# finalfusion/reductive

Hardware: AMD Instinct MI355X
Metric: vectors/sec PQ encode (d=300, M=15, K=256) (higher is better)
Workload: dtype f32

## Files before the change

reductive_amd/csrc/kernels_mfma16_screen.hip.h:

```cpp
#pragma once
#include "kernels_mfma.hip.h"

namespace pqhip {

constexpr float kScreenRel = 0x1.2p-9f;
constexpr float kScreenAbs = 0x1p-100f;
constexpr float kScreenTiny = 0x1p-100f;
constexpr int kScreenScaleLo = 12;
constexpr float kScreenMaxXX = 0x1p30f;
constexpr float kScreenMinCC = 0x1p-100f;

template <int T, int DP> constexpr bool mfma16_screens() { return mfma16_screen_shape(T, DP); }

constexpr int kScreenImageBytes = 256 * 32 * 2;
constexpr int kScreenHeaderBytes = 16;
constexpr size_t screen_image_bytes(int64_t M) { return (size_t)M * (kScreenImageBytes + kScreenHeaderBytes); }

struct ScreenScale {
    bool cc_range;
    float sc, sc2;
};
__device__ __forceinline__ ScreenScale screen_scale(float maxcc)
{
    ScreenScale r;
    r.cc_range = maxcc >= kScreenMinCC && maxcc < kBigNorm;
    const int escale = r.cc_range ? (kScreenScaleLo + 1 - ((int)(__float_as_uint(maxcc) >> 23) - 127)) >> 1 : 0;
    r.sc = __uint_as_float((unsigned)(127 + escale) << 23);
    r.sc2 = __uint_as_float((unsigned)(127 + 2 * escale) << 23);
    return r;
}

typedef _Float16 f16x8_t __attribute__((ext_vector_type(8)));
typedef _Float16 f16x2_t __attribute__((ext_vector_type(2)));
typedef unsigned u32x4_t __attribute__((ext_vector_type(4)));

__device__ __forceinline__ unsigned pk_f16(float a, float b)
{
    return __builtin_bit_cast(unsigned, __builtin_convertvector((f32x2){a, b}, f16x2_t));
}
__device__ __forceinline__ float f16_lo(unsigned p) { return (float)__builtin_bit_cast(f16x2_t, p)[0]; }
__device__ __forceinline__ float vmin(float a, float b) { float r; asm("v_min_f32 %0, %1, %2" : "=v"(r) : "v"(a), "v"(b)); return r; }
__device__ __forceinline__ float vmax(float a, float b) { float r; asm("v_max_f32 %0, %1, %2" : "=v"(r) : "v"(a), "v"(b)); return r; }
__device__ __forceinline__ void keep2(float& m, float& s, float k1, float k2)
{
    float t;
    asm("v_med3_f32 %0, %1, %2, %3" : "=v"(t) : "v"(m), "v"(k1), "v"(k2));
    asm("v_min_f32 %0, %0, %1" : "+v"(s) : "v"(t));
    asm("v_min3_f32 %0, %0, %1, %2" : "+v"(m) : "v"(k1), "v"(k2));
}
__device__ __forceinline__ float vmin3(float a, float b, float c) { float r; asm("v_min3_f32 %0, %1, %2, %3" : "=v"(r) : "v"(a), "v"(b), "v"(c)); return r; }
__device__ __forceinline__ void fold2(float& m, float a, float b) { asm("v_min3_f32 %0, %0, %1, %2" : "+v"(m) : "v"(a), "v"(b)); }

#define PQHIP_GLOBAL_AS __attribute__((address_space(1)))
#define PQHIP_LDS_AS __attribute__((address_space(3)))
typedef unsigned u32x2_t __attribute__((ext_vector_type(2)));
typedef f32x4_u PQHIP_GLOBAL_AS const* gf32x4_p;
__device__ __forceinline__ void load20_global(const PQHIP_GLOBAL_AS float* p, float (&v)[20])
{
#pragma unroll
    for (int e = 0; e < 20; e += 4) {
        const f32x4 t = *reinterpret_cast<gf32x4_p>(p + e);
        v[e] = t[0]; v[e + 1] = t[1]; v[e + 2] = t[2]; v[e + 3] = t[3];
    }
}
__device__ __forceinline__ float chain_dot20(const float (&a)[20], const float (&b)[20])
{
    float ab = 0.f;
#pragma unroll
    for (int k = 0; k < 20; ++k) ab = ffma(a[k], b[k], ab);
    return ab;
}

template <typename IdxT>
__device__ __forceinline__ void encode_rows_cand_f16(const float* x, int64_t x_rs, void* out, int64_t o_rs, const float* cbk,
                                                  const float* ccn, int K, int k_pad, int dsub, int64_t n, int m,
                                                  int64_t row_begin, const unsigned short* img, const unsigned* tiles,
                                                  unsigned long long flagged_c, float sc, float maxcct)
{
    constexpr int DP = 20, kRow = 32;
    const int lane = threadIdx.x & 63;
    const int i16 = lane & 15;
    const int q = lane >> 4;
    const int c0 = (8 * q) % 20, c1 = (8 * q + 4) % 20;
    const PQHIP_GLOBAL_AS float* const xsub = (const PQHIP_GLOBAL_AS float*)x + (int64_t)m * dsub;
    const PQHIP_GLOBAL_AS float* const plast = xsub + (n - 1) * x_rs;
    const PQHIP_GLOBAL_AS float* const cbm = (const PQHIP_GLOBAL_AS float*)cbk + (int64_t)m * K * DP;
    const PQHIP_GLOBAL_AS float* const ccm = (const PQHIP_GLOBAL_AS float*)ccn + (int64_t)m * k_pad;
    const PQHIP_LDS_AS unsigned* const tiles_l = (const PQHIP_LDS_AS unsigned*)tiles;
    const float sl = q < 3 ? sc : 0.f;
    const float sc2 = sc * sc;
    const PQHIP_LDS_AS unsigned short* const arow = (const PQHIP_LDS_AS unsigned short*)img + (i16 * kRow + 8 * (q ^ ((i16 >> 2) & 3)));
    unsigned cur = 0;
    int cur_ti = 0;
    while (cur || flagged_c) {
        int rel = -1;
        for (int t = 0; t < 16; ++t) {
            while (!cur && flagged_c) {
                cur_ti = __builtin_ctzll(flagged_c);
                flagged_c &= flagged_c - 1;
                cur = __builtin_amdgcn_readfirstlane(tiles_l[cur_ti]);
            }
            if (!cur) break;
            const int r = 32 * cur_ti + __builtin_ctz(cur);
            cur &= cur - 1;
            if (i16 == t) rel = r;
        }
        const bool rv = rel >= 0;
        const int64_t row = row_begin + rel;
        const PQHIP_GLOBAL_AS float* p = rv ? xsub + row * x_rs : plast;
        const f32x4 v0 = *reinterpret_cast<gf32x4_p>(p + c0), v1 = *reinterpret_cast<gf32x4_p>(p + c1);
        unsigned w[4] = {pk_f16(sl * v0[0], sl * v0[1]), pk_f16(sl * v0[2], sl * v0[3]), pk_f16(sl * v1[0], sl * v1[1]),
                         pk_f16(sl * v1[2], sl * v1[3])};
        if (q == 2) { w[2] = 0x3c003c00u; w[3] = 0x7bffu; }
        const u32x4_t bo = (u32x4_t){w[0], w[1], w[2], w[3]};
        float s0 = 0.f, s1 = 0.f;
#pragma unroll
        for (int j = 0; j < 4; ++j) { s0 = fmaf(v0[j], v0[j], s0); s1 = fmaf(v1[j], v1[j], s1); }
        float u[4];
        gather_groups((q < 3 ? s0 : 0.f) + (q < 2 ? s1 : 0.f), u);
        const float xxs = sc2 * ((u[0] + u[1]) + (u[2] + u[3]));
        auto block = [&](const PQHIP_LDS_AS unsigned short* ar, int cb) {
            const u32x4_t af = *reinterpret_cast<const PQHIP_LDS_AS u32x4_t*>(ar + cb * 16 * kRow);
            return __builtin_amdgcn_mfma_f32_16x16x32_f16(__builtin_bit_cast(f16x8_t, af), __builtin_bit_cast(f16x8_t, bo),
                                                          (f32x4){0.f, 0.f, 0.f, 0.f}, 0, 0, 0);
        };
        float mn = __builtin_inff();
#pragma unroll
        for (int cb = 0; cb < 16; ++cb) {
            if (cb % 4 == 0) __builtin_amdgcn_sched_barrier(0);
            const f32x4 d = block(arow, cb);
            mn = __builtin_elementwise_minimum(mn, __builtin_elementwise_minimum(__builtin_elementwise_minimum(d[0], d[1]),
                                                                                 __builtin_elementwise_minimum(d[2], d[3])));
        }
        float mq[4];
        gather_groups(mn, mq);
        const float tau = rv ? fminf(fminf(mq[0], mq[1]), fminf(mq[2], mq[3])) + (kScreenRel * (xxs + maxcct) + kScreenAbs)
                             : __builtin_nanf("");
        const PQHIP_LDS_AS unsigned short* arow2 = arow;
        asm volatile("" : "+v"(arow2) : "v"(tau));
        unsigned cw[2] = {0u, 0u};
#pragma unroll
        for (int cb = 0; cb < 16; ++cb) {
            if (cb % 4 == 0) __builtin_amdgcn_sched_barrier(0);
            const f32x4 d = block(arow2, cb);
#pragma unroll
            for (int v = 0; v < 4; ++v) cw[cb >> 3] |= (d[v] <= tau ? 1u : 0u) << (4 * (cb & 7) + v);
            if (cb % 4 == 3) asm volatile("" : "+v"(cw[cb >> 3]));
        }
        unsigned long long cm = ((unsigned long long)cw[1] << 32) | cw[0];
        float xr[DP];
        load20_global(xsub + (rv ? row : 0) * x_rs, xr);
        const float xxe = rv ? norm_unrolled_static<DP>(xr) : 0.f;
        unsigned bh = 0xffffffffu, bl = 0xffffffffu;
        while (__builtin_amdgcn_ballot_w64(cm != 0)) {
            int j[2];
            bool cv[2];
            float ce[2][DP], ccj[2];
#pragma unroll
            for (int s = 0; s < 2; ++s) {
                const int bit = cm ? __builtin_ctzll(cm) : 0;
                j[s] = 16 * (bit >> 2) + 4 * q + (bit & 3);
                cv[s] = cm != 0 && j[s] < K;
                cm &= cm - 1;
                const int jj = cv[s] ? j[s] : 0;
                load20_global(cbm + (int64_t)jj * DP, ce[s]);
                ccj[s] = ccm[jj];
            }
#pragma unroll
            for (int s = 0; s < 2; ++s) {
                const float dp = chain_dot20(xr, ce[s]);
                const unsigned kh = ord_key(fsub(fadd(xxe, ccj[s]), fadd(dp, dp)));
                if (cv[s] && (kh < bh || (kh == bh && (unsigned)j[s] < bl))) { bh = kh; bl = (unsigned)j[s]; }
            }
        }
        float hq[4], lq[4];
        gather_groups(__uint_as_float(bh), hq);
        gather_groups(__uint_as_float(bl), lq);
        bh = __float_as_uint(hq[0]);
        bl = __float_as_uint(lq[0]);
#pragma unroll
        for (int g = 1; g < 4; ++g) {
            const unsigned h = __float_as_uint(hq[g]), l = __float_as_uint(lq[g]);
            if (h < bh || (h == bh && l < bl)) { bh = h; bl = l; }
        }
        if (rv && q == 0) ((PQHIP_GLOBAL_AS IdxT*)out)[row * o_rs + m] = (IdxT)bl;
    }
}

constexpr int kScreenFewCap = 96;
constexpr int kScreenFewWords = 3;

template <typename IdxT>
__device__ __noinline__ void encode_rows_few(const float* x, int64_t x_rs, void* out, int64_t o_rs, const float* cbk,
                                             const float* ccn, int K, int k_pad, int dsub, int m, int64_t row_begin,
                                             const uint2* list, int count)
{
    constexpr int DP = 20;
    const int lane = threadIdx.x & 63;
    const PQHIP_GLOBAL_AS float* const xsub = (const PQHIP_GLOBAL_AS float*)x + (int64_t)m * dsub;
    const PQHIP_GLOBAL_AS float* const cbm = (const PQHIP_GLOBAL_AS float*)cbk + (int64_t)m * K * DP;
    const PQHIP_GLOBAL_AS float* const ccm = (const PQHIP_GLOBAL_AS float*)ccn + (int64_t)m * k_pad;
    const PQHIP_LDS_AS u32x2_t* const list_l = (const PQHIP_LDS_AS u32x2_t*)list;
    for (int e0 = 0; e0 < count; e0 += 64) {
        const bool rv = e0 + lane < count;
        const PQHIP_LDS_AS u32x2_t* const en = list_l + kScreenFewWords * (rv ? e0 + lane : 0);
        const u32x2_t w0 = en[0], w1 = en[1], w2 = en[2];
        const unsigned key[4] = {w0[0], w0[1], w1[0], w1[1]};
        const float tau = __uint_as_float(w2[0]);
        const int64_t row = row_begin + w2[1];
        float xr[DP];
        load20_global(xsub + row * x_rs, xr);
        const float xxe = norm_unrolled_static<DP>(xr);
        unsigned bh = 0xffffffffu, bl = 0xffffffffu;
#pragma unroll
        for (int g = 0; g < 4; ++g) {
            const unsigned kb = key[g] & 63u;
            const int j = (int)(16u * (kb >> 2) + 4u * g + (kb & 3u));
            const bool cg = __uint_as_float(key[g]) <= tau && j < K;
            const int jj = cg ? j : 0;
            float ce[DP];
            load20_global(cbm + (int64_t)jj * DP, ce);
            const float dp = chain_dot20(xr, ce);
            const unsigned kh = ord_key(fsub(fadd(xxe, ccm[jj]), fadd(dp, dp)));
            if (cg && (kh < bh || (kh == bh && (unsigned)j < bl))) { bh = kh; bl = (unsigned)j; }
        }
        if (rv) ((PQHIP_GLOBAL_AS IdxT*)out)[row * o_rs + m] = (IdxT)bl;
    }
}

template <typename IdxT>
__device__ __forceinline__ void encode_mfma16_screen(const EncodeArgs& a)
{
    constexpr int DP = 20;
    constexpr int kRow = 32;
    __shared__ __attribute__((aligned(16))) unsigned short img_s[256 * kRow];
    __shared__ unsigned need_s[4][kMfma16MaxTiles];
    __shared__ unsigned cand_s[4][kMfma16MaxTiles];
    __shared__ uint2 few_s[4][kScreenFewCap * kScreenFewWords];

    const int lane = threadIdx.x & 63;
    const int wave = __builtin_amdgcn_readfirstlane(threadIdx.x >> 6);
    const int i16 = lane & 15;
    const int q = lane >> 4;

    const int64_t b = blockIdx.x;
    const int xcd = (int)(b & 7);
    const int64_t qq = b >> 3;
    const int64_t g_local = qq / a.M;
    const int m = (int)(qq - g_local * a.M);
    const int64_t group = g_local * 8 + xcd;
    const bool wg_active = (g_local < a.chunks_per_xcd) && (group < a.n_chunks);

    const unsigned long long st_s0 = a.stamps ? __builtin_amdgcn_s_memtime() : 0;
    unsigned maxcc_bits = 0u;
    if (wg_active) {
        const u32x4_t* src = reinterpret_cast<const u32x4_t*>(a.screen_img) + (int64_t)m * (kScreenImageBytes / 16) + threadIdx.x;
        u32x4_t* dst = reinterpret_cast<u32x4_t*>(img_s) + threadIdx.x;
        u32x4_t ch[4];
#pragma unroll
        for (int j = 0; j < 4; ++j) ch[j] = src[256 * j];
        maxcc_bits = a.screen_img[(int64_t)a.M * (kScreenImageBytes / 4) + m * (kScreenHeaderBytes / 4)];
#pragma unroll
        for (int j = 0; j < 4; ++j) dst[256 * j] = ch[j];
    }
    const float maxcc = __uint_as_float(maxcc_bits);
    const ScreenScale scale = screen_scale(maxcc);
    const bool cc_range = scale.cc_range;
    const float sc = scale.sc, sc2 = scale.sc2;
    __syncthreads();
    const unsigned long long st_stage = a.stamps ? __builtin_amdgcn_s_memtime() - st_s0 : 0;
    const int64_t row_begin = (group * 4 + wave) * a.rows_per_item;
    if (!wg_active || row_begin >= a.n) return;
    int64_t row_end = row_begin + a.rows_per_item;
    if (row_end > a.n) row_end = a.n;
    const bool bad_codebook = a.bad_flag != nullptr && *a.bad_flag != 0;
    const bool near_rows = (uint64_t)a.x_rs < (1ull << 24) && (uint64_t)a.o_rs < (1ull << 24);
    const bool cb_ok = !bad_codebook && cc_range && near_rows;
    const float maxcct = sc2 * maxcc;

    const int c0 = (8 * q) % 20, c1 = (8 * q + 4) % 20;
    const float* const xsub = a.x + (int64_t)m * a.dsub;
    const unsigned xrs4 = near_rows ? (unsigned)a.x_rs * 4u : 0u;
    const unsigned xoff0 = (unsigned)i16 * xrs4 + 4u * c0, xoff1 = (unsigned)i16 * xrs4 + 4u * c1;
    const unsigned ooff = near_rows ? (unsigned)lane * (unsigned)a.o_rs * (unsigned)sizeof(IdxT) : 0u;
    auto load_rows = [&](float (&v)[8], const char* base, unsigned o0, unsigned o1) {
        asm volatile("" : "+v"(o0), "+v"(o1));
        const f32x4 v0 = *reinterpret_cast<const f32x4_u*>(base + o0), v1 = *reinterpret_cast<const f32x4_u*>(base + o1);
#pragma unroll
        for (int j = 0; j < 4; ++j) { v[j] = v0[j]; v[4 + j] = v1[j]; }
    };
    auto load_tile = [&](float (&v)[2][8], int64_t tile_row0) {
        if (tile_row0 + 32 <= a.n) {
            const char* base = reinterpret_cast<const char*>(xsub + tile_row0 * a.x_rs);
            load_rows(v[0], base, xoff0, xoff1);
            load_rows(v[1], base + 64 * a.x_rs, xoff0, xoff1);
        } else {
            const int64_t r0 = tile_row0 < a.n ? tile_row0 : a.n - 1;
            const int last = (int)(a.n - 1 - r0);
            const char* base = reinterpret_cast<const char*>(xsub + r0 * a.x_rs);
#pragma unroll
            for (int rb = 0; rb < 2; ++rb) {
                const unsigned ro = (unsigned)(16 * rb + i16 < last ? 16 * rb + i16 : last) * xrs4;
                load_rows(v[rb], base, ro + 4u * c0, ro + 4u * c1);
            }
        }
    };
    const float sl = q < 3 ? sc : 0.f;
    const bool tail = q == 2;
    auto split = [&](const float (&v)[2][8], u32x4_t (&bop)[2], float (&own)[2]) {
#pragma unroll
        for (int rb = 0; rb < 2; ++rb) {
            unsigned w[4];
#pragma unroll
            for (int j = 0; j < 4; ++j) w[j] = pk_f16(sl * v[rb][2 * j], sl * v[rb][2 * j + 1]);
            if (tail) { w[2] = 0x3c003c00u; w[3] = 0x7bffu; }
            bop[rb] = (u32x4_t){w[0], w[1], w[2], w[3]};
            float s0 = 0.f, s1 = 0.f;
#pragma unroll
            for (int j = 0; j < 4; ++j) { s0 = fmaf(v[rb][j], v[rb][j], s0); s1 = fmaf(v[rb][4 + j], v[rb][4 + j], s1); }
            own[rb] = (q < 3 ? s0 : 0.f) + (q < 2 ? s1 : 0.f);
        }
    };

    const unsigned kKeyMask = 0xffffffc0u, kBlockMask = 0xfffffff0u;
    unsigned long long flagged = 0, flagged_c = 0;
    uint2* few_w = few_s[wave];
    int few_room = kScreenFewCap;
    unsigned long long st_tiles = 0, st_steps = 0, st_rows = 0;
    unsigned long long st_full = 0;
    const unsigned long long st_t0 = a.stamps ? __builtin_amdgcn_s_memtime() : 0, st_r0 = a.stamps ? __builtin_amdgcn_s_memrealtime() : 0;
    const unsigned short* const arow = &img_s[i16 * kRow + 8 * (q ^ ((i16 >> 2) & 3))];
    auto load_a = [&](int cb, u32x4_t& af) { af = *reinterpret_cast<const u32x4_t*>(arow + cb * 16 * kRow); };
    auto screen2 = [&](const u32x4_t (&af)[2], const u32x4_t& b, f32x4 (&acc)[2]) {
#pragma unroll
        for (int j = 0; j < 2; ++j)
            acc[j] = __builtin_amdgcn_mfma_f32_16x16x32_f16(__builtin_bit_cast(f16x8_t, af[j]), __builtin_bit_cast(f16x8_t, b),
                                                            (f32x4){0.f, 0.f, 0.f, 0.f}, 0, 0, 0);
    };

    float xv[2][8];
    u32x4_t bop[2];
    float own[2];
    load_tile(xv, row_begin);
    split(xv, bop, own);
    u32x4_t af[2];
    f32x4 acc[2][2];
    load_a(0, af[0]);
    load_a(1, af[1]);
    screen2(af, bop[0], acc[0]);
    __builtin_amdgcn_sched_barrier(0);
    asm volatile("s_nop 7\n\ts_nop 7\n\ts_nop 7");
    __builtin_amdgcn_sched_barrier(0);
    auto tile = [&](int64_t row0, const u32x4_t (&bop)[2], u32x4_t (&bnext)[2], float (&ownn)[2], float (&mk)[2], float (&sk)[2]) {
        asm("" : "+s"(row0));
        load_tile(xv, row0 + 32);
        float mB[2], sB[2], mv[2][4];
#pragma unroll
        for (int p = 0; p < 8; ++p) {
#pragma unroll
            for (int rb = 0; rb < 2; ++rb) {
                if (rb == 0) {
                    screen2(af, bop[1], acc[1]);
                    load_a((2 * p + 2) & 15, af[0]);
                    load_a((2 * p + 3) & 15, af[1]);
                    if (p == 4) split(xv, bnext, ownn);
                } else {
                    screen2(af, p < 7 ? bop[0] : bnext[0], acc[0]);
                }
                __builtin_amdgcn_sched_barrier(0);
                const f32x4 d0 = acc[rb][0], d1 = acc[rb][1];
                const float b0 = vmin3(d0[0], d0[1], vmin(d0[2], d0[3])), b1 = vmin3(d1[0], d1[1], vmin(d1[2], d1[3]));
                const float k0 = __uint_as_float((__float_as_uint(b0) & kBlockMask) | (unsigned)(2 * p));
                const float k1 = __uint_as_float((__float_as_uint(b1) & kBlockMask) | (unsigned)(2 * p + 1));
                if (p == 0) {
                    mB[rb] = vmin(k0, k1);
                    sB[rb] = vmax(k0, k1);
#pragma unroll
                    for (int v = 0; v < 4; ++v) mv[rb][v] = vmin(d0[v], d1[v]);
                } else {
                    keep2(mB[rb], sB[rb], k0, k1);
#pragma unroll
                    for (int v = 0; v < 4; ++v) fold2(mv[rb][v], d0[v], d1[v]);
                }
            }
        }
#pragma unroll
        for (int rb = 0; rb < 2; ++rb) {
            float mA = vmin(mv[rb][0], mv[rb][1]), sA = vmax(mv[rb][0], mv[rb][1]);
            keep2(mA, sA, mv[rb][2], mv[rb][3]);
            unsigned vs = mv[rb][1] == mA ? 1u : 0u;
            vs = mv[rb][2] == mA ? 2u : vs;
            vs = mv[rb][3] == mA ? 3u : vs;
            const unsigned mb = __float_as_uint(mB[rb]);
            mk[rb] = __uint_as_float((mb & kKeyMask) | (((mb & 15u) << 2) | vs));
            sk[rb] = vmin(sA, sB[rb]);
        }
    };
    u32x4_t bop2[2];
    float own2[2], ownn[2] = {0.f, 0.f};
    float mk[2], sk[2], mk2[2], sk2[2];
    for (int64_t row0 = row_begin, tile_idx = 0; row0 < row_end; row0 += 64, tile_idx += 2) {
        const unsigned long long st_a = a.stamps ? __builtin_amdgcn_s_memtime() : 0;
        tile(row0, bop, bop2, own2, mk, sk);
        const bool two = row0 + 32 < row_end;
        if (two) tile(row0 + 32, bop2, bop, ownn, mk2, sk2);
        else mk2[0] = mk2[1] = sk2[0] = sk2[1] = __builtin_inff();
        float mq[4] = {mk[0], mk[1], mk2[0], mk2[1]}, sq[4] = {sk[0], sk[1], sk2[0], sk2[1]};
        float u[4] = {own[0], own[1], own2[0], own2[1]};
        transpose_groups(mq);
        transpose_groups(sq);
        transpose_groups(u);
        const float xx = sc2 * ((u[0] + u[1]) + (u[2] + u[3]));
        const float lo01 = vmin(mq[0], mq[1]), hi01 = vmax(mq[0], mq[1]);
        const float lo23 = vmin(mq[2], mq[3]), hi23 = vmax(mq[2], mq[3]);
        const float M = vmin(lo01, lo23);
        const float S2 = vmin(vmin(sq[0], sq[1]), vmin(sq[2], sq[3]));
        const float S = vmin(vmin(vmax(lo01, lo23), vmin(hi01, hi23)), S2);
        const float tau = M + (kScreenRel * (xx + maxcct) + kScreenAbs);
        const bool valid = lane < (int)(row_end - row0 < 64 ? row_end - row0 : 64);
        const bool in_range = valid && cb_ok && xx < kScreenMaxXX;
        const bool plain = in_range && __builtin_fabsf(M) > kScreenTiny;
        const bool one = plain && S > tau;
        if (one) {
            const unsigned Mb = __float_as_uint(M);
            const unsigned qw = Mb == __float_as_uint(lo01) ? (Mb == __float_as_uint(mq[0]) ? 0u : 1u)
                                                            : (Mb == __float_as_uint(mq[2]) ? 2u : 3u);
            const unsigned kb = Mb & 63u;
            char* ob = reinterpret_cast<char*>(reinterpret_cast<IdxT*>(a.out) + (row0 * a.o_rs + m));
            unsigned oo = ooff;
            asm volatile("" : "+v"(oo));
            *reinterpret_cast<IdxT*>(ob + oo) = (IdxT)(16 * (kb >> 2) + 4 * qw + (kb & 3));
        }
        const bool few = plain && !one && S2 > tau && (tau < -kScreenTiny || M > kScreenTiny);
        const unsigned long long fewm = __builtin_amdgcn_ballot_w64(few);
        const int pos = (int)__builtin_amdgcn_mbcnt_hi((unsigned)(fewm >> 32), __builtin_amdgcn_mbcnt_lo((unsigned)fewm, 0u));
        const bool listed = few && pos < few_room;
        if (listed) {
            uint2* const en = few_w + kScreenFewWords * pos;
            en[0] = make_uint2(__float_as_uint(mq[0]), __float_as_uint(mq[1]));
            en[1] = make_uint2(__float_as_uint(mq[2]), __float_as_uint(mq[3]));
            en[2] = make_uint2(__float_as_uint(tau), (unsigned)(row0 - row_begin) + (unsigned)lane);
        }
        const int few_k = __builtin_popcountll(fewm);
        few_w += kScreenFewWords * few_k;
        few_room -= few_k;
        const unsigned long long need = __builtin_amdgcn_ballot_w64(valid && !in_range);
        const unsigned long long cand = __builtin_amdgcn_ballot_w64(in_range && !one && !listed);
        auto record = [&](unsigned* rec, unsigned long long& tiles, unsigned long long rows) {
            const unsigned lo = (unsigned)rows, hi = (unsigned)(rows >> 32);
            if (lo) {
                if (lane == 0) rec[tile_idx] = lo;
                tiles |= 1ull << tile_idx;
            }
            if (hi) {
                if (lane == 0) rec[tile_idx + 1] = hi;
                tiles |= 2ull << tile_idx;
            }
        };
        record(need_s[wave], flagged, need);
        record(cand_s[wave], flagged_c, cand);
        if (a.stamps) {
            const int nfew = __builtin_popcountll(__builtin_amdgcn_ballot_w64(plain && !one && S2 > tau));
            const int off = __builtin_popcountll(need | __builtin_amdgcn_ballot_w64(in_range && !one));
            st_rows += (unsigned long long)nfew | ((unsigned long long)(off - nfew) << 32);
            st_full += (unsigned long long)__builtin_popcountll(__builtin_amdgcn_ballot_w64(few && !listed));
            st_tiles += two ? 2 : 1;
            st_steps += __builtin_amdgcn_s_memtime() - st_a;
        }
        own[0] = ownn[0];
        own[1] = ownn[1];
    }
    const unsigned long long st_p0 = a.stamps ? __builtin_amdgcn_s_memtime() : 0;
    if (few_room < kScreenFewCap)
        encode_rows_few<IdxT>(a.x, a.x_rs, a.out, a.o_rs, a.cb, a.cc, a.K, a.k_pad, a.dsub, m, row_begin, few_s[wave],
                              kScreenFewCap - (few_room > 0 ? few_room : 0));
    const unsigned long long st_p1 = a.stamps ? __builtin_amdgcn_s_memtime() : 0;
    if (flagged_c)
        encode_rows_cand_f16<IdxT>(a.x, a.x_rs, a.out, a.o_rs, a.cb, a.cc, a.K, a.k_pad, a.dsub, a.n, m, row_begin,
                                   img_s, cand_s[wave], flagged_c, sc, sc2 * maxcc);
    const unsigned long long st_p2 = a.stamps ? __builtin_amdgcn_s_memtime() : 0;
    while (flagged) {
        const int ti = __builtin_ctzll(flagged);
        flagged &= flagged - 1;
        const unsigned nd = __builtin_amdgcn_readfirstlane(need_s[wave][ti]);
        encode_rows_slow_v<IdxT, DP>(a.x, a.x_rs, a.out, a.o_rs, a.cb, a.cc, a.K, DP, a.k_pad, 0, m, row_begin + 32 * (int64_t)ti, nd);
    }
    if (a.stamps && lane == 0) {
        unsigned long long* o = a.stamps + ((size_t)blockIdx.x * 4 + wave) * kScreenStampWords;
        o[0] = st_tiles; o[1] = st_steps; o[2] = st_rows;
        const unsigned long long st_end = __builtin_amdgcn_s_memtime();
        o[3] = st_end - st_t0; o[4] = __builtin_amdgcn_s_memrealtime() - st_r0; o[5] = st_stage;
        o[6] = st_full; o[7] = st_end - st_p0;
        o[8] = st_p1 - st_p0; o[9] = st_p2 - st_p1;
    }
}

}
```

reductive_amd/csrc/pqhip_encode.hip:

```cpp
#include "pqhip_internal.h"

#include "kernels_anchor.hip.h"
#include "kernels_pair16.hip.h"
#include "encode_launch.h"
#include "opq_fused2_launch.h"
#include "smallk_launch.h"
#include "small16_launch.h"
#include "vor2_launch.h"
#include "wide_launch.h"

using namespace pqhip;

namespace pqh {

static EncodePlan planned(EncodeFamily f, const char* kernel) { EncodePlan p; p.family = f; p.kernel = kernel; return p; }
static EncodePlan unsupported() { EncodePlan p; p.status = PQHIP_EUNSUPPORTED; return p; }

static EncodePlan mfma_plan(const pqhip_codebook& cb, int kind)
{
    static const char* const names[2][3] = {{"k_encode_mfma<odd>", "k_encode_mfma<vec2>", "k_encode_mfma<vec4>"},
                                            {"k_encode_mfma_lds3<odd>", "k_encode_mfma_lds3<vec2>", "k_encode_mfma_lds3<vec4>"}};
    EncodePlan p = planned(EncodeFamily::mfma, "k_encode_mfma16");
    p.kind = kind; p.vec = cb.DP == cb.dsub; p.grp = (cb.DP % 4 == 0) ? 4 : 2;
    if (kind != 3) p.kernel = (!p.vec && cb.DP > 32) ? "k_encode_mfma_lds3<padded>" : names[kind / 2][p.vec ? p.grp / 2 : 0];
// ... 77 lines not shown
    const int64_t chunk = std::min<int64_t>(n, std::max<int64_t>(4096, (1ll << 30) / per_row));
    ScratchLease buf(cb, slot, io.st);
    PQCHK(buf.acquire((size_t)chunk * per_row));
    unsigned long long* keys = (unsigned long long*)buf.ptr();
    float* xx = (float*)(keys + chunk * Mv);
    const int64_t per_item = wide ? 1024 : 4096, rpi_max = wide ? 512 : 1024;
    for (int64_t r0 = 0; r0 < n; r0 += chunk) {
        const int64_t rows = std::min<int64_t>(chunk, n - r0);
        const float* x = io.x + r0 * io.x_rs;
        if (wide) { launch_row_norms(x, rows, io.x_rs, (int)cb->M, (int)cb->dsub, xx, io.st); note_kernel("k_row_norms"); }
        EncodeArgs a;
        a.x = x; a.n = rows; a.x_rs = io.x_rs; a.out = keys; a.o_rs = Mv;
        a.frags = cd.frags; a.cc = cd.cc; a.cb = cd.cb;
        a.M = (int)Mv; a.K = (int)cb->K; a.dsub = (int)cb->dsub; a.k_pad = cb->k_pad;
        a.groups = cb->groups; a.bad_flag = nullptr;
        const int64_t rpi = std::max<int64_t>(32, std::min<int64_t>(rpi_max, round_up((rows * Mv + 4 * per_item - 1) / (4 * per_item), 32)));
        a.rows_per_item = (int)rpi;
        a.n_chunks = (rows + 4 * rpi - 1) / (4 * rpi);
        a.chunks_per_xcd = (a.n_chunks + 7) / 8;
        const dim3 grid((unsigned)(a.chunks_per_xcd * Mv * 8));
        PQCHK(launched(wide ? launch_encode_wide(cb->T, cb->DP, a, xx, grid, io.st)
                            : launch_encode_mfma(2, 8, cb->DP, cb->DP == cb->dsub, 8, a, grid, io.st, diag().lds_pad),
                       p.kernel));
        note_kernel(p.kernel);
        const unsigned mg = (unsigned)std::min<int64_t>((rows * cb->M + 255) / 256, 256 * 32);
        if (c.code_bytes == 4)
            hipLaunchKernelGGL((k_merge_keys<uint32_t>), dim3(mg), dim3(256), 0, io.st, (const unsigned long long*)keys, rows, (int)cb->M,
                               cb->groups, (uint32_t*)io.codes + r0 * io.o_rs, io.o_rs);
        else
            hipLaunchKernelGGL((k_merge_keys<uint8_t>), dim3(mg), dim3(256), 0, io.st, (const unsigned long long*)keys, rows, (int)cb->M,
                               cb->groups, (uint8_t*)io.codes + r0 * io.o_rs, io.o_rs);
        HIPCHK(hipGetLastError());
        note_kernel("k_merge_keys");
    }
    return PQHIP_OK;
}

static int32_t launch_opq_fused(pqhip_codebook* cb, int slot, const EncodeCall& c, const EncodeIo& io)
{
    CodebookDev& cd = cb->dev[slot];
    const int DP = (int)cb->dsub;
    OpqFusedArgs a;
    a.x = io.x; a.n = c.n; a.x_rs = io.x_rs; a.P = cd.P; a.d = (int)cb->d;
    a.frags = cd.frags; a.cc = cd.cc; a.cb = cd.cb; a.out = (uint8_t*)io.codes; a.o_rs = io.o_rs;
    a.M = (int)cb->M; a.K = (int)cb->K; a.k_pad = cb->k_pad;
    const int nm = opq_fused2_slots(DP, cb->T, (int)cb->d) / DP;
    a.ncb = (int)((cb->M + nm - 1) / nm);
    const int64_t want_rg = std::max<int64_t>(1, 8ll * c.n_cus / a.ncb);
    const int f2_tiles = diag().fused2_tiles ? diag().fused2_tiles : (int)std::max<int64_t>(4, std::min<int64_t>(96, (c.n / want_rg + 255) / 256));
    a.rows_per_wg = 8 * 32 * f2_tiles;
    const int64_t n_rg = (c.n + a.rows_per_wg - 1) / a.rows_per_wg;
    a.rg_per_xcd = (n_rg + 7) / 8;
    const dim3 grid((unsigned)(a.rg_per_xcd * a.ncb * 8));
    StampRun stamps;
    PQCHK(stamps.begin(diag().fused_stamp, (size_t)grid.x * 8 * 5, io.st));
    a.stamps = stamps.ptr();
    const int e = launch_opq_fused2(DP, cb->T, a, grid, io.st);
    if (e < 0) return no_instantiation("k_opq_encode_fused2");
    if (e > 0) { g_hip_err = std::string("k_opq_encode_fused2: ") + hipGetErrorString((hipError_t)e); return PQHIP_EHIP; }
    return stamps.report5(io.st, "fused2", "rotation", "encode");
}

static int32_t launch_vor2_family(pqhip_codebook* cb, int slot, const EncodeCall& c, const EncodeIo& io)
{
    const CodebookDev& cd = cb->dev[slot];
    const Vor2Launch l{io.x, c.n, io.x_rs, (uint8_t*)io.codes, io.o_rs, cd.cb, cd.cc, cd.vor2_tab, cd.vor2_off,
                       (int)cb->M, (int)cb->K, cb->k_pad, (int)cb->dsub, cb->vor2_max_region_words, c.n_cus};
    return launched(launch_vor2(l, io.st), "k_encode_vor2");
}

template <int D>
static int32_t pair16(const Pair16Args& a, unsigned grid, size_t lds, hipStream_t st)
{
    if constexpr (!pair16_has(D)) {
        return PQHIP_EUNSUPPORTED;
    } else {
        HIPCHK(hipFuncSetAttribute((const void*)k_encode_pair16<D>, hipFuncAttributeMaxDynamicSharedMemorySize, 160 * 1024));
        hipLaunchKernelGGL((k_encode_pair16<D>), dim3(grid), dim3(256), lds, st, a);
        return PQHIP_OK;
    }
}

static int32_t launch_pair16(pqhip_codebook* cb, int slot, const EncodeCall& c, const EncodeIo& io)
{
    CodebookDev& cd = cb->dev[slot];
    Pair16Args a;
    const int NP = (int)((cb->M + 1) / 2);
    a.x = io.x; a.n = c.n; a.x_rs = io.x_rs; a.out = (uint8_t*)io.codes; a.o_rs = io.o_rs;
    a.fragp = cd.fragp; a.ccp = cd.fragp + (int64_t)NP * cb->dsub * 64; a.cb = cd.cb; a.cc = cd.cc;
    a.M = (int)cb->M; a.K = (int)cb->K; a.k_pad = cb->k_pad; a.NP = NP;
    a.n_tiles = (c.n + 31) / 32;
    const size_t lds = ((size_t)NP * cb->dsub * 64 + (size_t)NP * 32 + 4 * 2 * 32 * 36) * sizeof(float);
    const int per_cu = std::max<int>(1, std::min<int>(3, (int)(160 * 1024 / lds)));
    const unsigned grid = (unsigned)std::min<int64_t>((a.n_tiles + 3) / 4, (int64_t)c.n_cus * per_cu);
    const int32_t status = dispatch_int<1, 2, 4, 8, 16, 32>((int)cb->dsub, [&](auto d_c) { return pair16<decltype(d_c)::value>(a, grid, lds, io.st); });
    return status == PQHIP_EUNSUPPORTED ? no_instantiation("k_encode_pair16") : status;
}

static int32_t launch_small(pqhip_codebook* cb, int slot, const EncodePlan& p, const EncodeCall& c, const EncodeIo& io)
{
    CodebookDev& cd = cb->dev[slot];
    SmallKArgs a;
    a.x = io.x; a.n = c.n; a.x_rs = io.x_rs; a.out = (uint8_t*)io.codes; a.o_rs = io.o_rs;
    a.cbt = cd.cbt; a.cc = cd.cc; a.cb = cd.cb;
    a.M = (int)cb->M; a.K = (int)cb->K; a.k_pad = cb->k_pad;
    if (p.family == EncodeFamily::smallk)
        return launched(launch_smallk(cb->KP, (int)cb->dsub, a, dim3((unsigned)((c.n + 255) / 256)), io.st), p.kernel);
    const int64_t tile_rows = small16_tile_rows((int)cb->dsub);
    const int64_t n_tiles = (c.n + tile_rows - 1) / tile_rows;
    const int64_t wg_slots = (int64_t)c.n_cus * 4 * 8;
    a.word_stores = c.word_codes ? 1 : 0;
    a.tiles_per_wave = (int)std::max<int64_t>(1, std::min<int64_t>(kSmall16TilesMax, n_tiles / (4 * wg_slots)));
    const size_t lds = small16_lds_bytes(a.M, (int)cb->dsub, cb->KP);
    const dim3 grid((unsigned)((n_tiles + 4 * a.tiles_per_wave - 1) / (4 * a.tiles_per_wave)));
    return launched(launch_small16(cb->KP, (int)cb->dsub, a, grid, lds, io.st), p.kernel);
}

static int32_t launch_mfma(pqhip_codebook* cb, int slot, const EncodePlan& p, const EncodeCall& c, const EncodeIo& io)
{
    CodebookDev& cd = cb->dev[slot];
    const int64_t n = c.n;
    EncodeArgs a;
    a.x = io.x; a.n = n; a.x_rs = io.x_rs; a.out = io.codes; a.o_rs = io.o_rs;
    a.frags = cd.frags; a.cc = cd.cc; a.cb = cd.cb;
    a.M = (int)cb->M; a.K = (int)cb->K; a.dsub = (int)cb->dsub; a.k_pad = cb->k_pad;
    a.groups = 1; a.bad_flag = io.bad_flag;
    a.screen_img = cd.screen_img;
    if (p.kind == 3 && mfma16_screen_shape(cb->T, cb->DP)) {
        if (!a.screen_img) return no_instantiation("k_encode_mfma16 (no screen image)");
        if (cd.screen_img_stale) PQCHK(build_screen_image(cb, slot, io.st));
    }
    dim3 grid;
    if (p.kind >= 2) {
        const int64_t rpi_max = diag().rpi_max, rpi_min = diag().rpi_min;
        int64_t rpi = round_up((n * cb->M + 4 * 4096 - 1) / (4 * 4096), 32);
        rpi = std::max<int64_t>(rpi_min, std::min<int64_t>(rpi_max, rpi));
        if (p.kind == 3) rpi = std::min<int64_t>(rpi, 32 * kMfma16MaxTiles);
        a.rows_per_item = (int)rpi;
        a.n_chunks = (n + 4 * rpi - 1) / (4 * rpi);
        a.chunks_per_xcd = (a.n_chunks + 7) / 8;
        grid = dim3((unsigned)(a.chunks_per_xcd * cb->M * 8));
    } else {
        const int64_t rpi = std::max<int64_t>(32, std::min<int64_t>(1024, round_up((n * cb->M + 4095) / 4096, 32)));
        a.rows_per_item = (int)rpi;
        a.n_chunks = (n + rpi - 1) / rpi;
        a.chunks_per_xcd = (a.n_chunks + 7) / 8;
        grid = dim3((unsigned)((a.chunks_per_xcd * cb->M + 3) / 4 * 8));
    }
    StampRun stamps;
    const int stamp_words = (p.kind == 3 && mfma16_screen_shape(cb->T, cb->DP)) ? kScreenStampWords : 5;
    PQCHK(stamps.begin(diag().enc_stamp && p.kind >= 2, (size_t)grid.x * 4 * stamp_words, io.st));
    a.stamps = stamps.ptr();
    PQCHK(launched(launch_encode_mfma(p.kind, cb->T, cb->DP, p.vec, c.code_bytes, a, grid, io.st, diag().lds_pad), p.kernel));
    if (p.kind == 3) return stamps.report5(io.st, "encode", "steps", "2-4-candidate / other off-screen", true, stamp_words);
    return stamps.report5(io.st, "encode", "steps", "seam");
}

static int32_t launch_anchor(pqhip_codebook* cb, int slot, const EncodeCall& c, const EncodeIo& io)
{
    CodebookDev& cd = cb->dev[slot];
    const unsigned grid = (unsigned)std::min<int64_t>((c.n * cb->M + 255) / 256, 256 * 32);
    if (c.code_bytes == 1)
        hipLaunchKernelGGL((k_encode_scalar<uint8_t>), dim3(grid), dim3(256), 0, io.st, io.x, c.n, io.x_rs, (uint8_t*)io.codes, io.o_rs, cd.cb,
                           cd.cc, (int)cb->M, (int)cb->K, (int)cb->dsub, cb->k_pad);
    else
        hipLaunchKernelGGL((k_encode_scalar<uint32_t>), dim3(grid), dim3(256), 0, io.st, io.x, c.n, io.x_rs, (uint32_t*)io.codes, io.o_rs,
                           cd.cb, cd.cc, (int)cb->M, (int)cb->K, (int)cb->dsub, cb->k_pad);
    return PQHIP_OK;
}

int32_t encode_planned(pqhip_codebook* cb, int slot, const EncodePlan& p, const EncodeCall& c, const EncodeIo& io)
{
    if (p.status != PQHIP_OK) return p.status;
    switch (p.family) {
    case EncodeFamily::wide: case EncodeFamily::grouped: PQCHK(launch_keyed(cb, slot, p, c, io)); break;
    case EncodeFamily::opq_fused: PQCHK(launch_opq_fused(cb, slot, c, io)); break;
    case EncodeFamily::vor2: PQCHK(launch_vor2_family(cb, slot, c, io)); break;
    case EncodeFamily::pair16: PQCHK(launch_pair16(cb, slot, c, io)); break;
    case EncodeFamily::small16: case EncodeFamily::smallk: PQCHK(launch_small(cb, slot, p, c, io)); break;
    case EncodeFamily::mfma: PQCHK(launch_mfma(cb, slot, p, c, io)); break;
    case EncodeFamily::anchor: PQCHK(launch_anchor(cb, slot, c, io)); break;
    default: return no_instantiation("(no encode kernel planned)");
    }
    HIPCHK(hipGetLastError());
    if (p.family != EncodeFamily::wide && p.family != EncodeFamily::grouped) note_kernel(p.kernel);
    cb->last_kernel = p.kernel;
    return PQHIP_OK;
}

int32_t encode_plain_dev(pqhip_codebook* cb, int slot, const float* d_x, int64_t n, int64_t x_rs,
                         void* d_codes, int code_bytes, int64_t o_rs, hipStream_t st,
                         const int* bad_flag, bool beside_update)
{
    if (n == 0) return PQHIP_OK;
    const EncodeIo io{d_x, x_rs, d_codes, o_rs, st, bad_flag};
    EncodeCall c = encode_call(cb, slot, io, n, code_bytes);
    c.beside_update = beside_update;
    return encode_planned(cb, slot, plan_encode(*cb, c, cb->ctx->opt), c, io);
}

}
```

Before: 2.239 billion.

## Switch PQ screen kernel from 16x16x32 to 32x32x16 MFMA with half-wave candidate keys

Reworks the screening pass to use 32x32x16 f16 MFMAs. Each half-wave now covers 32 rows and 16 centroid columns per block, replacing the four-quarter 16x16 layout with two row blocks. The min/second-min reduction changes from a four-group transpose to a permlane32 swap. Fallback candidate entries shrink from three to two 8-byte words, written and read as one 16-byte LDS access. The aim is fewer MFMA issues, fewer shuffles and less LDS traffic per tile, at the cost of wider accumulators and a coarser candidate key that could send more rows to fallback.

```diff
diff --git a/reductive_amd/csrc/kernels_mfma16_screen.hip.h b/reductive_amd/csrc/kernels_mfma16_screen.hip.h
--- a/reductive_amd/csrc/kernels_mfma16_screen.hip.h
+++ b/reductive_amd/csrc/kernels_mfma16_screen.hip.h
@@ -9,6 +9,8 @@
 constexpr int kScreenScaleLo = 12;
 constexpr float kScreenMaxXX = 0x1p30f;
 constexpr float kScreenMinCC = 0x1p-100f;
+constexpr unsigned kKey7Mask = 0xffffff80u;
+[[maybe_unused]] constexpr unsigned kKeyMask = 0xffffffc0u;
 
 template <int T, int DP> constexpr bool mfma16_screens() { return mfma16_screen_shape(T, DP); }
 
@@ -188,7 +190,12 @@
 }
 
 constexpr int kScreenFewCap = 96;
-constexpr int kScreenFewWords = 3;
+constexpr int kScreenFewWords = 2;
+
+__device__ __forceinline__ unsigned screen_key_centroid(unsigned kb, unsigned h)
+{
+    return 16u * (kb >> 3) + 8u * ((kb >> 2) & 1u) + 4u * h + (kb & 3u);
+}
 
 template <typename IdxT>
 __device__ __noinline__ void encode_rows_few(const float* x, int64_t x_rs, void* out, int64_t o_rs, const float* cbk,
@@ -200,22 +207,20 @@
     const PQHIP_GLOBAL_AS float* const xsub = (const PQHIP_GLOBAL_AS float*)x + (int64_t)m * dsub;
     const PQHIP_GLOBAL_AS float* const cbm = (const PQHIP_GLOBAL_AS float*)cbk + (int64_t)m * K * DP;
     const PQHIP_GLOBAL_AS float* const ccm = (const PQHIP_GLOBAL_AS float*)ccn + (int64_t)m * k_pad;
-    const PQHIP_LDS_AS u32x2_t* const list_l = (const PQHIP_LDS_AS u32x2_t*)list;
+    const PQHIP_LDS_AS u32x4_t* const list_l = (const PQHIP_LDS_AS u32x4_t*)list;
     for (int e0 = 0; e0 < count; e0 += 64) {
         const bool rv = e0 + lane < count;
-        const PQHIP_LDS_AS u32x2_t* const en = list_l + kScreenFewWords * (rv ? e0 + lane : 0);
-        const u32x2_t w0 = en[0], w1 = en[1], w2 = en[2];
-        const unsigned key[4] = {w0[0], w0[1], w1[0], w1[1]};
-        const float tau = __uint_as_float(w2[0]);
-        const int64_t row = row_begin + w2[1];
+        const u32x4_t en = list_l[rv ? e0 + lane : 0];
+        const unsigned key[2] = {en[0], en[1]};
+        const float tau = __uint_as_float(en[2]);
+        const int64_t row = row_begin + en[3];
         float xr[DP];
         load20_global(xsub + row * x_rs, xr);
         const float xxe = norm_unrolled_static<DP>(xr);
         unsigned bh = 0xffffffffu, bl = 0xffffffffu;
 #pragma unroll
-        for (int g = 0; g < 4; ++g) {
-            const unsigned kb = key[g] & 63u;
-            const int j = (int)(16u * (kb >> 2) + 4u * g + (kb & 3u));
+        for (int g = 0; g < 2; ++g) {
+            const int j = (int)screen_key_centroid(key[g] & 127u, (unsigned)g);
             const bool cg = __uint_as_float(key[g]) <= tau && j < K;
             const int jj = cg ? j : 0;
             float ce[DP];
@@ -236,12 +241,12 @@
     __shared__ __attribute__((aligned(16))) unsigned short img_s[256 * kRow];
     __shared__ unsigned need_s[4][kMfma16MaxTiles];
     __shared__ unsigned cand_s[4][kMfma16MaxTiles];
-    __shared__ uint2 few_s[4][kScreenFewCap * kScreenFewWords];
+    __shared__ __attribute__((aligned(16))) uint2 few_s[4][kScreenFewCap * kScreenFewWords];
 
     const int lane = threadIdx.x & 63;
     const int wave = __builtin_amdgcn_readfirstlane(threadIdx.x >> 6);
-    const int i16 = lane & 15;
-    const int q = lane >> 4;
+    const int n32 = lane & 31;
+    const int h = lane >> 5;
 
     const int64_t b = blockIdx.x;
     const int xcd = (int)(b & 7);
@@ -278,144 +283,127 @@
     const bool cb_ok = !bad_codebook && cc_range && near_rows;
     const float maxcct = sc2 * maxcc;
 
-    const int c0 = (8 * q) % 20, c1 = (8 * q + 4) % 20;
     const float* const xsub = a.x + (int64_t)m * a.dsub;
     const unsigned xrs4 = near_rows ? (unsigned)a.x_rs * 4u : 0u;
-    const unsigned xoff0 = (unsigned)i16 * xrs4 + 4u * c0, xoff1 = (unsigned)i16 * xrs4 + 4u * c1;
-    const unsigned ooff = near_rows ? (unsigned)lane * (unsigned)a.o_rs * (unsigned)sizeof(IdxT) : 0u;
-    auto load_rows = [&](float (&v)[8], const char* base, unsigned o0, unsigned o1) {
-        asm volatile("" : "+v"(o0), "+v"(o1));
-        const f32x4 v0 = *reinterpret_cast<const f32x4_u*>(base + o0), v1 = *reinterpret_cast<const f32x4_u*>(base + o1);
-#pragma unroll
-        for (int j = 0; j < 4; ++j) { v[j] = v0[j]; v[4 + j] = v1[j]; }
-    };
-    auto load_tile = [&](float (&v)[2][8], int64_t tile_row0) {
+    const unsigned ors = near_rows ? (unsigned)a.o_rs * (unsigned)sizeof(IdxT) : 0u;
+    const unsigned xoff0 = (unsigned)n32 * xrs4 + 32u * (unsigned)h;
+    auto load_rows = [&](float (&v)[12], const char* base, unsigned o0) {
+        asm volatile("" : "+v"(o0));
+        const unsigned o1 = h ? o0 : o0 + 64u;
+        const f32x4 v0 = *reinterpret_cast<const f32x4_u*>(base + o0), v1 = *reinterpret_cast<const f32x4_u*>(base + o0 + 16);
+        const f32x4 v2 = *reinterpret_cast<const f32x4_u*>(base + o1);
+#pragma unroll
+        for (int j = 0; j < 4; ++j) { v[j] = v0[j]; v[4 + j] = v1[j]; v[8 + j] = v2[j]; }
+    };
+    auto load_tile = [&](float (&v)[12], int64_t tile_row0) {
         if (tile_row0 + 32 <= a.n) {
-            const char* base = reinterpret_cast<const char*>(xsub + tile_row0 * a.x_rs);
-            load_rows(v[0], base, xoff0, xoff1);
-            load_rows(v[1], base + 64 * a.x_rs, xoff0, xoff1);
+            load_rows(v, reinterpret_cast<const char*>(xsub + tile_row0 * a.x_rs), xoff0);
         } else {
             const int64_t r0 = tile_row0 < a.n ? tile_row0 : a.n - 1;
-            const int last = (int)(a.n - 1 - r0);
-            const char* base = reinterpret_cast<const char*>(xsub + r0 * a.x_rs);
-#pragma unroll
-            for (int rb = 0; rb < 2; ++rb) {
-                const unsigned ro = (unsigned)(16 * rb + i16 < last ? 16 * rb + i16 : last) * xrs4;
-                load_rows(v[rb], base, ro + 4u * c0, ro + 4u * c1);
-            }
-        }
-    };
-    const float sl = q < 3 ? sc : 0.f;
-    const bool tail = q == 2;
-    auto split = [&](const float (&v)[2][8], u32x4_t (&bop)[2], float (&own)[2]) {
-#pragma unroll
-        for (int rb = 0; rb < 2; ++rb) {
-            unsigned w[4];
-#pragma unroll
-            for (int j = 0; j < 4; ++j) w[j] = pk_f16(sl * v[rb][2 * j], sl * v[rb][2 * j + 1]);
-            if (tail) { w[2] = 0x3c003c00u; w[3] = 0x7bffu; }
-            bop[rb] = (u32x4_t){w[0], w[1], w[2], w[3]};
-            float s0 = 0.f, s1 = 0.f;
-#pragma unroll
-            for (int j = 0; j < 4; ++j) { s0 = fmaf(v[rb][j], v[rb][j], s0); s1 = fmaf(v[rb][4 + j], v[rb][4 + j], s1); }
-            own[rb] = (q < 3 ? s0 : 0.f) + (q < 2 ? s1 : 0.f);
-        }
-    };
-
-    const unsigned kKeyMask = 0xffffffc0u, kBlockMask = 0xfffffff0u;
+            int last = (int)(a.n - 1 - r0);
+            asm volatile("" : "+s"(last));
+            const int nl = lane & 31;
+            load_rows(v, reinterpret_cast<const char*>(xsub + r0 * a.x_rs), (unsigned)(nl < last ? nl : last) * xrs4 + (h ? 32u : 0u));
+        }
+    };
+    auto split = [&](const float (&v)[12], u32x4_t (&bop)[2], float& own) {
+        unsigned w[4];
+#pragma unroll
+        for (int j = 0; j < 4; ++j) w[j] = pk_f16(sc * v[2 * j], sc * v[2 * j + 1]);
+        bop[0] = (u32x4_t){w[0], w[1], w[2], w[3]};
+        const unsigned t0 = pk_f16(sc * v[8], sc * v[9]), t1 = pk_f16(sc * v[10], sc * v[11]);
+        bop[1] = (u32x4_t){h ? 0u : t0, h ? 0u : t1, h ? 0u : 0x3c003c00u, h ? 0u : 0x7bffu};
+        float s0 = 0.f, s1 = 0.f, s2 = 0.f;
+#pragma unroll
+        for (int j = 0; j < 4; ++j) { s0 = fmaf(v[j], v[j], s0); s1 = fmaf(v[4 + j], v[4 + j], s1); s2 = fmaf(v[8 + j], v[8 + j], s2); }
+        own = (s0 + s1) + (h ? 0.f : s2);
+    };
+
+    const unsigned kHalfMask = 0xfffffff0u, kColMask = 0xfffffff8u;
     unsigned long long flagged = 0, flagged_c = 0;
     uint2* few_w = few_s[wave];
     int few_room = kScreenFewCap;
     unsigned long long st_tiles = 0, st_steps = 0, st_rows = 0;
     unsigned long long st_full = 0;
     const unsigned long long st_t0 = a.stamps ? __builtin_amdgcn_s_memtime() : 0, st_r0 = a.stamps ? __builtin_amdgcn_s_memrealtime() : 0;
-    const unsigned short* const arow = &img_s[i16 * kRow + 8 * (q ^ ((i16 >> 2) & 3))];
-    auto load_a = [&](int cb, u32x4_t& af) { af = *reinterpret_cast<const u32x4_t*>(arow + cb * 16 * kRow); };
-    auto screen2 = [&](const u32x4_t (&af)[2], const u32x4_t& b, f32x4 (&acc)[2]) {
-#pragma unroll
-        for (int j = 0; j < 2; ++j)
-            acc[j] = __builtin_amdgcn_mfma_f32_16x16x32_f16(__builtin_bit_cast(f16x8_t, af[j]), __builtin_bit_cast(f16x8_t, b),
-                                                            (f32x4){0.f, 0.f, 0.f, 0.f}, 0, 0, 0);
-    };
-
-    float xv[2][8];
+    const unsigned short* const arow0 = &img_s[n32 * kRow + 8 * (h ^ ((n32 >> 2) & 3))];
+    const unsigned short* const arow1 = &img_s[n32 * kRow + 8 * ((2 + h) ^ ((n32 >> 2) & 3))];
+    auto load_a = [&](int b, u32x4_t (&af)[2]) {
+        af[0] = *reinterpret_cast<const u32x4_t*>(arow0 + b * 32 * kRow);
+        af[1] = *reinterpret_cast<const u32x4_t*>(arow1 + b * 32 * kRow);
+    };
+    auto screen = [&](const u32x4_t (&af)[2], const u32x4_t (&b)[2], f32x16& acc) {
+        const f32x16 z = {0.f, 0.f, 0.f, 0.f, 0.f, 0.f, 0.f, 0.f, 0.f, 0.f, 0.f, 0.f, 0.f, 0.f, 0.f, 0.f};
+        const f32x16 t = __builtin_amdgcn_mfma_f32_32x32x16_f16(__builtin_bit_cast(f16x8_t, af[0]), __builtin_bit_cast(f16x8_t, b[0]), z, 0, 0, 0);
+        acc = __builtin_amdgcn_mfma_f32_32x32x16_f16(__builtin_bit_cast(f16x8_t, af[1]), __builtin_bit_cast(f16x8_t, b[1]), t, 0, 0, 0);
+    };
+
+    float xv[12];
     u32x4_t bop[2];
-    float own[2];
+    float own;
     load_tile(xv, row_begin);
     split(xv, bop, own);
     u32x4_t af[2];
-    f32x4 acc[2][2];
-    load_a(0, af[0]);
-    load_a(1, af[1]);
-    screen2(af, bop[0], acc[0]);
+    f32x16 acc[2];
+    load_a(0, af);
+    screen(af, bop, acc[0]);
     __builtin_amdgcn_sched_barrier(0);
-    asm volatile("s_nop 7\n\ts_nop 7\n\ts_nop 7");
+    asm volatile("s_nop 7\n\ts_nop 7\n\ts_nop 7\n\ts_nop 7");
     __builtin_amdgcn_sched_barrier(0);
-    auto tile = [&](int64_t row0, const u32x4_t (&bop)[2], u32x4_t (&bnext)[2], float (&ownn)[2], float (&mk)[2], float (&sk)[2]) {
+    auto tile = [&](int64_t row0, const u32x4_t (&bop)[2], u32x4_t (&bnext)[2], float& ownn, float& mk, float& sk) {
         asm("" : "+s"(row0));
-        load_tile(xv, row0 + 32);
-        float mB[2], sB[2], mv[2][4];
-#pragma unroll
-        for (int p = 0; p < 8; ++p) {
-#pragma unroll
-            for (int rb = 0; rb < 2; ++rb) {
-                if (rb == 0) {
-                    screen2(af, bop[1], acc[1]);
-                    load_a((2 * p + 2) & 15, af[0]);
-                    load_a((2 * p + 3) & 15, af[1]);
-                    if (p == 4) split(xv, bnext, ownn);
-                } else {
-                    screen2(af, p < 7 ? bop[0] : bnext[0], acc[0]);
-                }
-                __builtin_amdgcn_sched_barrier(0);
-                const f32x4 d0 = acc[rb][0], d1 = acc[rb][1];
-                const float b0 = vmin3(d0[0], d0[1], vmin(d0[2], d0[3])), b1 = vmin3(d1[0], d1[1], vmin(d1[2], d1[3]));
-                const float k0 = __uint_as_float((__float_as_uint(b0) & kBlockMask) | (unsigned)(2 * p));
-                const float k1 = __uint_as_float((__float_as_uint(b1) & kBlockMask) | (unsigned)(2 * p + 1));
-                if (p == 0) {
-                    mB[rb] = vmin(k0, k1);
-                    sB[rb] = vmax(k0, k1);
-#pragma unroll
-                    for (int v = 0; v < 4; ++v) mv[rb][v] = vmin(d0[v], d1[v]);
-                } else {
-                    keep2(mB[rb], sB[rb], k0, k1);
-#pragma unroll
-                    for (int v = 0; v < 4; ++v) fold2(mv[rb][v], d0[v], d1[v]);
-                }
-            }
-        }
-#pragma unroll
-        for (int rb = 0; rb < 2; ++rb) {
-            float mA = vmin(mv[rb][0], mv[rb][1]), sA = vmax(mv[rb][0], mv[rb][1]);
-            keep2(mA, sA, mv[rb][2], mv[rb][3]);
-            unsigned vs = mv[rb][1] == mA ? 1u : 0u;
-            vs = mv[rb][2] == mA ? 2u : vs;
-            vs = mv[rb][3] == mA ? 3u : vs;
-            const unsigned mb = __float_as_uint(mB[rb]);
-            mk[rb] = __uint_as_float((mb & kKeyMask) | (((mb & 15u) << 2) | vs));
-            sk[rb] = vmin(sA, sB[rb]);
-        }
+        float mB, sB, mv[8];
+#pragma unroll
+        for (int b = 0; b < 8; ++b) {
+            load_a((b + 1) & 7, af);
+            if (b == 1) load_tile(xv, row0 + 32);
+            if (b == 5) split(xv, bnext, ownn);
+            screen(af, b < 7 ? bop : bnext, acc[(b + 1) & 1]);
+            __builtin_amdgcn_sched_barrier(0);
+            const f32x16 d = acc[b & 1];
+            const float b0 = vmin3(vmin3(d[0], d[1], d[2]), vmin3(d[3], d[4], d[5]), vmin(d[6], d[7]));
+            const float b1 = vmin3(vmin3(d[8], d[9], d[10]), vmin3(d[11], d[12], d[13]), vmin(d[14], d[15]));
+            const float k0 = __uint_as_float((__float_as_uint(b0) & kHalfMask) | (unsigned)(2 * b));
+            const float k1 = __uint_as_float((__float_as_uint(b1) & kHalfMask) | (unsigned)(2 * b + 1));
+            if (b == 0) {
+                mB = vmin(k0, k1);
+                sB = vmax(k0, k1);
+#pragma unroll
+                for (int c = 0; c < 8; ++c) mv[c] = vmin(d[c], d[8 + c]);
+            } else {
+                keep2(mB, sB, k0, k1);
+#pragma unroll
+                for (int c = 0; c < 8; ++c) fold2(mv[c], d[c], d[8 + c]);
+            }
+        }
+        float kv[8];
+#pragma unroll
+        for (int c = 0; c < 8; ++c) kv[c] = __uint_as_float((__float_as_uint(mv[c]) & kColMask) | (unsigned)c);
+        float mA = vmin(kv[0], kv[1]), sA = vmax(kv[0], kv[1]);
+        keep2(mA, sA, kv[2], kv[3]);
+        keep2(mA, sA, kv[4], kv[5]);
+        keep2(mA, sA, kv[6], kv[7]);
+        const unsigned mb = __float_as_uint(mB);
+        mk = __uint_as_float((mb & kKey7Mask) | (((mb & 15u) << 3) | (__float_as_uint(mA) & 7u)));
+        sk = vmin(sA, sB);
     };
     u32x4_t bop2[2];
-    float own2[2], ownn[2] = {0.f, 0.f};
-    float mk[2], sk[2], mk2[2], sk2[2];
+    float own2, ownn = 0.f;
+    float mk, sk, mk2, sk2;
     for (int64_t row0 = row_begin, tile_idx = 0; row0 < row_end; row0 += 64, tile_idx += 2) {
         const unsigned long long st_a = a.stamps ? __builtin_amdgcn_s_memtime() : 0;
         tile(row0, bop, bop2, own2, mk, sk);
         const bool two = row0 + 32 < row_end;
         if (two) tile(row0 + 32, bop2, bop, ownn, mk2, sk2);
-        else mk2[0] = mk2[1] = sk2[0] = sk2[1] = __builtin_inff();
-        float mq[4] = {mk[0], mk[1], mk2[0], mk2[1]}, sq[4] = {sk[0], sk[1], sk2[0], sk2[1]};
-        float u[4] = {own[0], own[1], own2[0], own2[1]};
-        transpose_groups(mq);
-        transpose_groups(sq);
-        transpose_groups(u);
-        const float xx = sc2 * ((u[0] + u[1]) + (u[2] + u[3]));
-        const float lo01 = vmin(mq[0], mq[1]), hi01 = vmax(mq[0], mq[1]);
-        const float lo23 = vmin(mq[2], mq[3]), hi23 = vmax(mq[2], mq[3]);
-        const float M = vmin(lo01, lo23);
-        const float S2 = vmin(vmin(sq[0], sq[1]), vmin(sq[2], sq[3]));
-        const float S = vmin(vmin(vmax(lo01, lo23), vmin(hi01, hi23)), S2);
+        else mk2 = sk2 = __builtin_inff();
+        const auto xm = __builtin_amdgcn_permlane32_swap(__float_as_uint(mk), __float_as_uint(mk2), false, false);
+        const auto xs = __builtin_amdgcn_permlane32_swap(__float_as_uint(sk), __float_as_uint(sk2), false, false);
+        const auto xu = __builtin_amdgcn_permlane32_swap(__float_as_uint(own), __float_as_uint(own2), false, false);
+        const float m0 = __uint_as_float(xm[0]), m1 = __uint_as_float(xm[1]);
+        const float xx = sc2 * (__uint_as_float(xu[0]) + __uint_as_float(xu[1]));
+        const float M = vmin(m0, m1);
+        const float S2 = vmin(__uint_as_float(xs[0]), __uint_as_float(xs[1]));
+        const float S = vmin(vmax(m0, m1), S2);
         const float tau = M + (kScreenRel * (xx + maxcct) + kScreenAbs);
         const bool valid = lane < (int)(row_end - row0 < 64 ? row_end - row0 : 64);
         const bool in_range = valid && cb_ok && xx < kScreenMaxXX;
@@ -423,24 +411,21 @@
         const bool one = plain && S > tau;
         if (one) {
             const unsigned Mb = __float_as_uint(M);
-            const unsigned qw = Mb == __float_as_uint(lo01) ? (Mb == __float_as_uint(mq[0]) ? 0u : 1u)
-                                                            : (Mb == __float_as_uint(mq[2]) ? 2u : 3u);
-            const unsigned kb = Mb & 63u;
+            const unsigned hw = Mb == __float_as_uint(m0) ? 0u : 1u;
             char* ob = reinterpret_cast<char*>(reinterpret_cast<IdxT*>(a.out) + (row0 * a.o_rs + m));
-            unsigned oo = ooff;
+            unsigned os = ors;
+            asm volatile("" : "+s"(os));
+            unsigned oo = (unsigned)lane * os;
             asm volatile("" : "+v"(oo));
-            *reinterpret_cast<IdxT*>(ob + oo) = (IdxT)(16 * (kb >> 2) + 4 * qw + (kb & 3));
+            *reinterpret_cast<IdxT*>(ob + oo) = (IdxT)screen_key_centroid(Mb & 127u, hw);
         }
         const bool few = plain && !one && S2 > tau && (tau < -kScreenTiny || M > kScreenTiny);
         const unsigned long long fewm = __builtin_amdgcn_ballot_w64(few);
         const int pos = (int)__builtin_amdgcn_mbcnt_hi((unsigned)(fewm >> 32), __builtin_amdgcn_mbcnt_lo((unsigned)fewm, 0u));
         const bool listed = few && pos < few_room;
-        if (listed) {
-            uint2* const en = few_w + kScreenFewWords * pos;
-            en[0] = make_uint2(__float_as_uint(mq[0]), __float_as_uint(mq[1]));
-            en[1] = make_uint2(__float_as_uint(mq[2]), __float_as_uint(mq[3]));
-            en[2] = make_uint2(__float_as_uint(tau), (unsigned)(row0 - row_begin) + (unsigned)lane);
-        }
+        if (listed)
+            *reinterpret_cast<u32x4_t*>(few_w + kScreenFewWords * pos) =
+                (u32x4_t){__float_as_uint(m0), __float_as_uint(m1), __float_as_uint(tau), (unsigned)(row0 - row_begin) + (unsigned)lane};
         const int few_k = __builtin_popcountll(fewm);
         few_w += kScreenFewWords * few_k;
         few_room -= few_k;
@@ -467,8 +452,7 @@
             st_tiles += two ? 2 : 1;
             st_steps += __builtin_amdgcn_s_memtime() - st_a;
         }
-        own[0] = ownn[0];
-        own[1] = ownn[1];
+        own = ownn;
     }
     const unsigned long long st_p0 = a.stamps ? __builtin_amdgcn_s_memtime() : 0;
     if (few_room < kScreenFewCap)
diff --git a/reductive_amd/csrc/pqhip_encode.hip b/reductive_amd/csrc/pqhip_encode.hip
--- a/reductive_amd/csrc/pqhip_encode.hip
+++ b/reductive_amd/csrc/pqhip_encode.hip
@@ -253,7 +253,7 @@
     PQCHK(stamps.begin(diag().enc_stamp && p.kind >= 2, (size_t)grid.x * 4 * stamp_words, io.st));
     a.stamps = stamps.ptr();
     PQCHK(launched(launch_encode_mfma(p.kind, cb->T, cb->DP, p.vec, c.code_bytes, a, grid, io.st, diag().lds_pad), p.kernel));
-    if (p.kind == 3) return stamps.report5(io.st, "encode", "steps", "2-4-candidate / other off-screen", true, stamp_words);
+    if (p.kind == 3) return stamps.report5(io.st, "encode", "steps", "one-per-half / other off-screen", true, stamp_words);
     return stamps.report5(io.st, "encode", "steps", "seam");
 }
 
```

Measured after the change: 2.376 billion (median of 6 runs). 1.06x the previous value.
